# nizepart/Research-and-Development-of-Kubernetes-Operator-for-Machine-Learning-Pipelines

Measured on AMD Instinct MI355X. Metric: served_tokens_per_sec, higher is better.
Workload: dtype bf16

## Files before the change

### research-and-development-of-kubernetes-operator-for-machine-learning-pipelines_amd/ops/csrc/bindings.cpp

```cpp
#include <climits>
#include <cstdlib>
#include <string>
#include <torch/library.h>
#include <ATen/ATen.h>
#include <c10/hip/HIPStream.h>
#include <c10/core/DeviceGuard.h>
#include <cmath>

#include "launch.h"
#include "gemm_plan.h"

namespace {

using at::Tensor;

hipStream_t cur_stream() { return c10::hip::getCurrentHIPStream().stream(); }

void check_bf16(const Tensor& t, const char* name) {
  TORCH_CHECK(t.is_cuda(), name, " must be a GPU tensor");
  TORCH_CHECK(t.scalar_type() == at::kBFloat16, name, " must be bf16");
  TORCH_CHECK(t.is_contiguous(), name, " must be contiguous");
}
void check_i32(const Tensor& t, const char* name) {
  TORCH_CHECK(t.is_cuda(), name, " must be a GPU tensor");
// ... 403 lines not shown
std::vector<int64_t> gemm_route_env(int64_t M, int64_t N, int64_t K, int64_t op, int64_t cus, bool sk,
                                    int64_t n_groups, int64_t rows_per_group) {
  mlop::PlanEnv env = mlop::gemm_knobs();
  env.cus = (int)cus, env.sk = sk;
  return route_list(env, M, N, K, op, n_groups, rows_per_group);
}
std::vector<int64_t> gemm_tile_configs() {
  std::vector<int64_t> v;
  for (const mlop::TileCfg& t : mlop::kGemmTiles) v.insert(v.end(), {t.BM, t.BN, t.WM, t.WN, t.stages, t.setprio, t.rope});
  return v;
}

void check_a(const Tensor& a) {
  TORCH_CHECK(a.is_cuda() && a.scalar_type() == at::kBFloat16 && a.dim() == 2 && a.stride(1) == 1 &&
                  a.stride(0) % 8 == 0, "a must be bf16 [M, K], 16-B aligned rows");
}

mlop::RopeEpi rope_args(const Tensor& q_out, const Tensor& k_cache, const Tensor& v_cache, const Tensor& a,
                        const Tensor& w, const Tensor& pos, const Tensor& cos_sin, const Tensor& slots) {
  check_a(a);
  check_bf16(w, "w"); check_bf16(q_out, "q_out"); check_bf16(k_cache, "k_cache");
  check_bf16(v_cache, "v_cache"); check_i32(pos, "pos"); check_i32(slots, "slots");
  TORCH_CHECK(cos_sin.is_cuda() && cos_sin.scalar_type() == at::kFloat && cos_sin.is_contiguous(),
              "cos_sin f32");
  const int64_t M = a.size(0), K = a.size(1), N = w.size(0);
  TORCH_CHECK(w.dim() == 2 && w.size(1) == K && K % 64 == 0, "w [N, K], K % 64");
  TORCH_CHECK(q_out.dim() == 3 && k_cache.dim() == 4 && v_cache.dim() == 4, "ranks");
  const int64_t Hq = q_out.size(1), D = q_out.size(2), Hkv = k_cache.size(1), BS = k_cache.size(2);
  TORCH_CHECK(D == 128 && k_cache.size(3) == D && v_cache.sizes() == k_cache.sizes(),
              "head_dim 128; k and v [NB,Hkv,BS,D]");
  TORCH_CHECK(N == (Hq + 2 * Hkv) * D && q_out.size(0) == M, "qkv width / q_out rows");
  TORCH_CHECK(pos.numel() == M && slots.numel() == M, "pos/slots length");
  TORCH_CHECK(cos_sin.dim() == 2 && cos_sin.size(1) == D, "cos_sin [max_pos, D]");
  return mlop::RopeEpi{(uint16_t*)q_out.data_ptr(), (uint16_t*)k_cache.data_ptr(),
                       (uint16_t*)v_cache.data_ptr(), pos.data_ptr<int>(), cos_sin.data_ptr<float>(),
                       slots.data_ptr<int>(), (int)Hq, (int)Hkv, (int)BS};
}

void gemm(Tensor out, Tensor a, Tensor w, Tensor ws, int64_t epi) {
  TORCH_CHECK(a.is_cuda() && a.scalar_type() == at::kBFloat16 && a.dim() == 2 && a.stride(1) == 1,
              "a must be bf16 [M, K] with unit inner stride");
  check_bf16(w, "w");
  TORCH_CHECK(out.is_cuda() && out.scalar_type() == at::kBFloat16 && out.dim() == 2 &&
                  out.stride(1) == 1, "out must be bf16 [M, N]");
  const int64_t M = a.size(0), K = a.size(1), N = w.size(0);
  TORCH_CHECK(w.dim() == 2 && w.size(1) == K, "w must be [N, K]");
  TORCH_CHECK(K % 64 == 0, "K must be a multiple of 64");
  TORCH_CHECK(N % 8 == 0 && a.stride(0) % 8 == 0 && out.stride(0) % 8 == 0, "16-B aligned rows");
  TORCH_CHECK(epi == 0 || epi == 1, "epi");
  TORCH_CHECK(epi == 0 || N % 32 == 0, "silu_mul epilogue needs N % 32 == 0");
  TORCH_CHECK(out.size(0) == M && out.size(1) == (epi == 0 ? N : N / 2), "out shape");
  TORCH_CHECK(reinterpret_cast<uintptr_t>(a.data_ptr()) % 16 == 0 &&
                  reinterpret_cast<uintptr_t>(out.data_ptr()) % 16 == 0, "16-B aligned data");
  float* wsp = nullptr;
  int64_t wsn = 0;
  if (ws.defined() && ws.numel() > 0) {
    TORCH_CHECK(ws.is_cuda() && ws.scalar_type() == at::kFloat, "ws f32");
    wsp = ws.data_ptr<float>();
    wsn = ws.numel();
  }
  c10::DeviceGuard g(a.device());
  mlop::launch_gemm(a.data_ptr(), (int)a.stride(0), w.data_ptr(), (int)K, out.data_ptr(),
                    (int)out.stride(0), wsp, wsn, (int)M, (int)N, (int)K, (int)epi, cur_stream());
}

bool gemm_rope_cache(Tensor q_out, Tensor k_cache, Tensor v_cache, Tensor a, Tensor w, Tensor pos,
                     Tensor cos_sin, Tensor slots) {
  const mlop::RopeEpi re = rope_args(q_out, k_cache, v_cache, a, w, pos, cos_sin, slots);
  c10::DeviceGuard g(a.device());
// ... 16 lines not shown
  TORCH_CHECK(N % 128 == 0, "N % 128");
  check_ss(ss_out, M, N, "ss");
  c10::DeviceGuard g(a.device());
  return mlop::launch_gemm_chain(mlop::OP_CHAIN_RES_SS, a.data_ptr(), (int)a.stride(0), w.data_ptr(),
                                 residual.data_ptr(), (int)residual.stride(0), (int)M, (int)N, (int)K,
                                 mlop::RopeEpi{}, ss_out.data_ptr<float>(), 0.f, cur_stream());
}

bool gemm_rs(Tensor out, Tensor a, Tensor w, Tensor ss_in, double eps, int64_t epi) {
  check_a(a);
  check_bf16(w, "w"); check_bf16(out, "out");
  const int64_t M = a.size(0), K = a.size(1), N = w.size(0);
  TORCH_CHECK(w.dim() == 2 && w.size(1) == K, "w [N, K]");
  TORCH_CHECK(epi == 0 || epi == 1, "epi");
  TORCH_CHECK(out.dim() == 2 && out.size(0) == M && out.size(1) == (epi == 0 ? N : N / 2) && out.stride(1) == 1 &&
                  out.stride(0) % 8 == 0, "out [M, N or N/2]");
  TORCH_CHECK(K % 128 == 0, "K % 128");
  check_ss(ss_in, M, K, "ss");
  c10::DeviceGuard g(a.device());
  return mlop::launch_gemm_chain(mlop::OP_CHAIN_RS | (int)epi, a.data_ptr(), (int)a.stride(0), w.data_ptr(),
                                 out.data_ptr(), (int)out.stride(0), (int)M, (int)N, (int)K, mlop::RopeEpi{},
                                 ss_in.data_ptr<float>(), (float)eps, cur_stream());
}

bool gemm_rs_rope(Tensor q_out, Tensor k_cache, Tensor v_cache, Tensor a, Tensor w, Tensor pos, Tensor cos_sin,
                  Tensor slots, Tensor ss_in, double eps) {
  const mlop::RopeEpi re = rope_args(q_out, k_cache, v_cache, a, w, pos, cos_sin, slots);
  const int64_t M = a.size(0), K = a.size(1), N = w.size(0);
  TORCH_CHECK(K % 128 == 0, "K % 128");
  check_ss(ss_in, M, K, "ss");
  c10::DeviceGuard g(a.device());
  return mlop::launch_gemm_chain(mlop::OP_CHAIN_RS_ROPE, a.data_ptr(), (int)a.stride(0), w.data_ptr(), nullptr, 0,
                                 (int)M, (int)N, (int)K, re, ss_in.data_ptr<float>(), (float)eps, cur_stream());
}

bool gemm_add_rmsnorm(Tensor out, Tensor residual, Tensor a, Tensor w, Tensor norm_w, Tensor ws,
                      double eps) {
  check_a(a);
  check_bf16(w, "w"); check_bf16(out, "out"); check_bf16(residual, "residual");
  check_bf16(norm_w, "norm_w");
  const int64_t M = a.size(0), K = a.size(1), N = w.size(0);
  TORCH_CHECK(w.size(1) == K && K % 64 == 0 && N % 8 == 0, "w [N, K], K % 64");
  TORCH_CHECK(out.numel() == M * N && residual.numel() == M * N && norm_w.numel() == N, "shapes");
  TORCH_CHECK(ws.is_cuda() && ws.scalar_type() == at::kFloat, "ws f32");
  c10::DeviceGuard g(a.device());
  return mlop::launch_gemm_add_rmsnorm(a.data_ptr(), (int)a.stride(0), w.data_ptr(), out.data_ptr(),
                                       residual.data_ptr(), norm_w.data_ptr(), (float)eps,
                                       ws.data_ptr<float>(), ws.numel(), (int)M, (int)N, (int)K,
                                       cur_stream());
}

bool gemm_ws(Tensor out, Tensor a, Tensor w, int64_t epi, bool rs, double eps) {
  check_a(a);
  check_bf16(w, "w"); check_bf16(out, "out");
  const int64_t M = a.size(0), K = a.size(1), N = w.size(0);
  TORCH_CHECK(w.dim() == 2 && w.size(1) == K && w.stride(0) == K, "w [N, K] contiguous");
  TORCH_CHECK(epi == 0 || epi == 1 || epi == 5, "epi 0 / 1 / 5");
  TORCH_CHECK(out.dim() == 2 && out.size(0) == M && out.size(1) == (epi == 1 ? N / 2 : N) && out.stride(1) == 1,
              "out [M, N or N/2]");
  TORCH_CHECK(!(rs && epi == 5), "residual form has no row scale");
  if (!mlop::ws_takes(mlop::gemm_live_env(), (int)M, (int)N, (int)K, (int)epi)) return false;
  c10::DeviceGuard g(a.device());
  mlop::launch_ws(a.data_ptr(), (int)a.stride(0), w.data_ptr(), (int)K, out.data_ptr(), (int)out.stride(0), (int)M,
                  (int)N, (int)K, (int)epi, rs, mlop::RopeEpi{}, (float)eps, cur_stream());
  return true;
}
// ... 561 lines not shown
  m.def("decode_chain_max_m() -> int", &decode_chain_max_m);
  m.def("gemm_ws_plan(int rb, int u, int nt) -> ()", &gemm_ws_plan);
  m.def("gemm_ws_small_m(int set=-1) -> int", &knob<mlop::gemm_ws_small_m>);
  m.def("gemm_ws_rope_m(int set=-1) -> int", &knob<mlop::gemm_ws_rope_m>);
  m.def("flash_persist(int set=-1) -> int", &knob<mlop::flash_persist>);
  m.def("flash_stream(int set=-1) -> int", &knob<mlop::flash_stream>);
  m.def("gemm_grouped_balance(int set=-1) -> int", &knob<mlop::gemm_grouped_balance>);
  m.def("gemm_grouped_order(int set=-1) -> int", &knob<mlop::gemm_grouped_order>);
  m.def("moe_mid_tok(int set=-1) -> int", &knob<mlop::moe_mid_tok>);
  m.def("gemm_mid_chain(int set=-1) -> int", &knob<mlop::gemm_mid_chain>);
  m.def("mid_chain_ok(int M, int N, int K, int epi) -> bool", &mid_chain_ok);
  m.def("moe_mid_max_tokens(int set=-1) -> int", &knob<mlop::moe_mid_max_tokens>);
  m.def("gemm_grouped_plan(int bm, int bn, int stages, int splits) -> ()", &gemm_grouped_plan);
  m.def("gemm_dense_plan(int variant, int bm, int bn, int splits, int stages=0) -> ()", &gemm_dense_plan);
  m.def("gemm_small_stages(int set=-1) -> int", &knob<mlop::gemm_small_stages>);
  m.def("gemm_small_tile(int set=-1) -> int", &knob<mlop::gemm_small_tile>);
  m.def("gemm_sk_mode(int set=-1) -> int", &knob<mlop::gemm_sk_mode>);
  m.def("gemm_sk_reserve() -> bool", &gemm_sk_reserve);
  m.def("gemm_sk_workgroups(int M, int N, int K) -> int", &gemm_sk_workgroups);
  m.def("vmm_supported(int device) -> bool", &vmm_supported);
  m.def("vmm_granularity(int device) -> int", &vmm_granularity);
  m.def("vmm_arena(int bytes, int device) -> Tensor", &vmm_arena);
  m.def("vmm_map_chunks(Tensor flat, int region_stride, int n_regions, int chunk_bytes, int first, "
        "int count, bool async_) -> bool", &vmm_map_chunks);
  m.def("vmm_chunks_ready(Tensor flat) -> int", &vmm_chunks_ready);
  m.def("vmm_error(Tensor flat) -> int", &vmm_error);
  m.def("gemm_rope_supported(int M, int N, int K) -> bool", &gemm_rope_supported);
  m.def("w4_chain_ok(int M, int N, int K) -> bool", &w4_chain_ok);
  m.def("chain_ok(int M, int N, int K, int epi) -> bool", &chain_ok);
  m.def("gemm_route(int M, int N, int K, int op, int n_groups=0, int rows_per_group=0) -> int[]", &gemm_route);
  m.def("gemm_route_env(int M, int N, int K, int op, int cus, bool sk, int n_groups=0, int rows_per_group=0) -> int[]", &gemm_route_env);
  m.def("gemm_tile_configs() -> int[]", &gemm_tile_configs);
  m.def("gemm_res_ss(Tensor(a!) residual, Tensor a, Tensor w, Tensor(b!) ss_out) -> bool");
  m.def("gemm_rs(Tensor(a!) out, Tensor a, Tensor w, Tensor ss_in, float eps, int epi) -> bool");
  m.def("gemm_rs_rope(Tensor(a!) q_out, Tensor(b!) k_cache, Tensor(c!) v_cache, Tensor a, Tensor w, "
        "Tensor pos, Tensor cos_sin, Tensor slots, Tensor ss_in, float eps) -> bool");
  m.def("gemm_rope_cache(Tensor(a!) q_out, Tensor(b!) k_cache, Tensor(c!) v_cache, Tensor a, Tensor w, "
        "Tensor pos, Tensor cos_sin, Tensor slots) -> bool");
  m.def("gemm(Tensor(a!) out, Tensor a, Tensor w, Tensor(b!) ws, int epi) -> ()");
  m.def("grouped_gemm(Tensor(a!) out, Tensor a, Tensor w, Tensor offsets, int max_rows, "
        "int epi, Tensor? a_rows=None) -> ()");
  m.def("gemm_add_rmsnorm(Tensor(a!) out, Tensor(b!) residual, Tensor a, Tensor w, Tensor norm_w, "
        "Tensor(c!) ws, float eps) -> bool");
  m.def("gemv_chain_supported(int M, int N, int K, int epi) -> bool", &gemv_chain_supported);
  m.def("moe_route(Tensor(a!) topw, Tensor(b!) topi, Tensor logits) -> ()");
  m.def("moe_permute(Tensor(a!) xp, Tensor(b!) offsets, Tensor(c!) src, Tensor(d!) inv, Tensor x, "
        "Tensor topi, int e0, int n_local) -> ()");
  m.def("moe_combine(Tensor(a!) out, Tensor y, Tensor inv, Tensor topw) -> ()");
  m.def("moe_dispatch_small(Tensor(a!) topw, Tensor(b!) topi, Tensor(c!) xp, Tensor(d!) offsets, Tensor(e!) src, "
        "Tensor(f!) inv, Tensor(g!) x, Tensor router_w, int e0, int n_local, Tensor? pro_y=None, "
        "Tensor(h!)? pro_res=None, Tensor? pro_w=None, float pro_eps=0.0) -> bool");
  m.def("moe_dispatch_mid(Tensor(a!) topw, Tensor(b!) topi, Tensor(c!) offsets, Tensor(d!) arow, Tensor(e!) inv, "
        "Tensor(f!) x, Tensor router_w, int e0, int n_local, Tensor? pro_y=None, Tensor(g!)? pro_res=None, "
        "Tensor? pro_w=None, float pro_eps=0.0) -> bool");
  m.def("moe_down_combine_add_rmsnorm(Tensor(a!) out, Tensor(b!) residual, Tensor(c!) y, Tensor a, Tensor w2, "
        "Tensor offsets, int max_rows, Tensor inv, Tensor topw, Tensor norm_w, float eps) -> bool");
  m.def("moe_combine_add_rmsnorm(Tensor(a!) out, Tensor(b!) residual, Tensor y, Tensor inv, Tensor topw, "
        "Tensor norm_w, float eps) -> bool");
  m.def("argmax(Tensor(a!) out, Tensor logits) -> ()");
  m.def("sample(Tensor(a!) out, Tensor logits, Tensor temps, Tensor top_ks, Tensor top_ps, "
        "Tensor uniform, bool full) -> ()");
  m.def("penalty_reset(Tensor(a!) table, int slot, int vocab, Tensor prompt_ids, Tensor output_ids) -> ()");
  m.def("penalty_update(Tensor(a!) table, int vocab, Tensor slots, Tensor tokens) -> ()");
  m.def("grammar_mask(Tensor(a!) logits, Tensor arena, Tensor base, Tensor rows, Tensor state) -> ()");
  m.def("grammar_advance(Tensor arena, int vocab, Tensor base, Tensor rows, Tensor(a!) state, Tensor tokens) -> ()");
  m.def("apply_penalties(Tensor(a!) logits, Tensor table, Tensor slots, Tensor rep, Tensor freq, "
// ... 24 lines not shown
        "int nparts, int window=0) -> ()");
  m.def("rope_cache_fp8(Tensor(a!) q_out, Tensor(b!) k_cache, Tensor(c!) v_cache, Tensor(d!) k_scale, "
        "Tensor(e!) v_scale, Tensor qkv, Tensor pos, Tensor cos_sin, Tensor slots) -> ()");
  m.def("rope_cache_qkn(Tensor(a!) q_out, Tensor(b!) k_cache, Tensor(c!) v_cache, Tensor qkv, Tensor pos, "
        "Tensor cos_sin, Tensor slots, Tensor q_w, Tensor k_w, float eps) -> ()");
  m.def("rope_cache_qkn_fp8(Tensor(a!) q_out, Tensor(b!) k_cache, Tensor(c!) v_cache, Tensor(d!) k_scale, "
        "Tensor(e!) v_scale, Tensor qkv, Tensor pos, Tensor cos_sin, Tensor slots, Tensor q_w, Tensor k_w, "
        "float eps) -> ()");
  m.def("paged_attention_fp8(Tensor(a!) out, Tensor(b!) part_o, Tensor(c!) part_ml, Tensor(d!) part_sem, Tensor q, "
        "Tensor k_cache, Tensor v_cache, Tensor k_scale, Tensor v_scale, Tensor block_tables, Tensor tile_seq, "
        "Tensor tile_q0, Tensor q_start, Tensor q_len, Tensor ctx_len, float scale, int part_tokens, "
        "int nparts) -> ()");
}

TORCH_LIBRARY_IMPL(mlop, CUDA, m) {
  m.impl("rmsnorm", &rmsnorm);
  m.impl("add_rmsnorm", &add_rmsnorm);
  m.impl("rope_cache", &rope_cache);
  m.impl("silu_mul", &silu_mul);
  m.impl("embedding", &embedding);
  m.impl("lora_shrink", &lora_shrink);
  m.impl("lora_expand_add", &lora_expand_add);
  m.impl("paged_attention", &paged_attention);
  m.impl("rope_cache_fp8", &rope_cache_fp8);
  m.impl("rope_cache_qkn", &rope_cache_qkn);
  m.impl("rope_cache_qkn_fp8", &rope_cache_qkn_fp8);
  m.impl("paged_attention_fp8", &paged_attention_fp8);
  m.impl("flash_prefill", &flash_prefill);
  m.impl("gemm", &gemm);
  m.impl("gemm_ws", &gemm_ws);
  m.impl("grouped_gemm", &grouped_gemm);
  m.impl("gemm_add_rmsnorm", &gemm_add_rmsnorm);
  m.impl("gemm_res_ss", &gemm_res_ss);
  m.impl("gemm_rs", &gemm_rs);
  m.impl("gemm_rs_rope", &gemm_rs_rope);
  m.impl("gemm_rope_cache", &gemm_rope_cache);
  m.impl("moe_route", &moe_route);
  m.impl("moe_dispatch_small", &moe_dispatch_small);
  m.impl("moe_dispatch_mid", &moe_dispatch_mid);
  m.impl("moe_down_combine_add_rmsnorm", &moe_down_combine_add_rmsnorm);
  m.impl("moe_combine_add_rmsnorm", &moe_combine_add_rmsnorm);
  m.impl("moe_permute", &moe_permute);
  m.impl("moe_combine", &moe_combine);
  m.impl("argmax", &argmax);
  m.impl("sample", &sample);
  m.impl("penalty_reset", &penalty_reset);
  m.impl("penalty_update", &penalty_update);
  m.impl("grammar_mask", &grammar_mask);
  m.impl("grammar_advance", &grammar_advance);
  m.impl("apply_penalties", &apply_penalties);
  m.impl("token_logprobs", &token_logprobs);
  m.impl("spec_accept", &spec_accept);
  m.impl("spec_propose", &spec_propose);
  m.impl("pool_accumulate", &pool_accumulate);
  m.impl("pool_finish", &pool_finish);
  m.impl("car_all_reduce", &car_all_reduce);
  m.impl("car_all_reduce_add", &car_all_reduce_add);
  m.impl("car_broadcast", &car_broadcast);
  m.impl("car_all_gather", &car_all_gather);
  m.impl("ep_dispatch", &ep_dispatch);
  m.impl("ep_combine", &ep_combine);
}
```

### research-and-development-of-kubernetes-operator-for-machine-learning-pipelines_amd/ops/csrc/gemm_w4.hip

```cpp
#include "common.h"
#include "launch.h"
#include "gemm_plan.h"
#include "gemm_w4_asm.h"

#include <type_traits>
#include <utility>

namespace mlop {

namespace {
enum { W4_NONE = 0, W4_SILU_MUL = 1, W4_ROPE = 3, W4_ADD_SS = 4, W4_RS = 8 };
using i32x4 = __attribute__((ext_vector_type(4))) int;
typedef __attribute__((address_space(3))) uint16_t lds_u16;

__device__ __forceinline__ i32x4 make_srd(const void* p) {
  const uint64_t a = (uint64_t)p;
  i32x4 r;
  r.x = __builtin_amdgcn_readfirstlane((int)(uint32_t)a);
  r.y = __builtin_amdgcn_readfirstlane((int)(uint32_t)(a >> 32));
  r.z = 0x7fffffff;
  r.w = 0x00020000;
  return r;
}

// ... 142 lines not shown
#define MLOP_W4H_OPERANDS                                                                                        \
  : [fa0_0] "=&v"(fa0_0), [fa0_1] "=&v"(fa0_1), [fa0_2] "=&v"(fa0_2), [fa0_3] "=&v"(fa0_3),                      \
    [fb0_0] "=&v"(fb0_0), [fb0_1] "=&v"(fb0_1), [fb0_2] "=&v"(fb0_2), [fb0_3] "=&v"(fb0_3),                      \
    [fb0_4] "=&v"(fb0_4), [fb0_5] "=&v"(fb0_5), [fb0_6] "=&v"(fb0_6), [fb0_7] "=&v"(fb0_7),                      \
    [fa1_0] "=&v"(fa1_0), [fa1_1] "=&v"(fa1_1), [fa1_2] "=&v"(fa1_2), [fa1_3] "=&v"(fa1_3),                      \
    [fb1_0] "=&v"(fb1_0), [fb1_1] "=&v"(fb1_1), [fb1_2] "=&v"(fb1_2), [fb1_3] "=&v"(fb1_3),                      \
    [fb1_4] "=&v"(fb1_4), [fb1_5] "=&v"(fb1_5), [fb1_6] "=&v"(fb1_6), [fb1_7] "=&v"(fb1_7),                      \
    [rA0] "+v"(rA0), [rA1] "+v"(rA1), [rB0] "+v"(rB0), [rB1] "+v"(rB1), [koff] "+s"(koff), [dbase] "+s"(dbase), \
    [iter] "+s"(iter), [m0save] "=&s"(m0save)                                                                    \
  : [vo0] "v"(vo[0]), [vo1] "v"(vo[1]), [vo2] "v"(vo[2]), [vo3] "v"(vo[3]), [vo4] "v"(vo[4]), [vo5] "v"(vo[5]), \
    [vo6] "v"(vo[6]), [vo7] "v"(vo[7]), [vo8] "v"(vo[8]), [vo9] "v"(vo[9]), [vo10] "v"(vo[10]),                 \
    [vo11] "v"(vo[11]), [vn0] "v"(vn[0]), [vn1] "v"(vn[1]), [vn2] "v"(vn[2]), [vn3] "v"(vn[3]),                 \
    [vn4] "v"(vn[4]), [vn5] "v"(vn[5]), [vn6] "v"(vn[6]), [vn7] "v"(vn[7]), [vn8] "v"(vn[8]), [vn9] "v"(vn[9]), \
    [vn10] "v"(vn[10]), [vn11] "v"(vn[11]), [srdA] "s"(srdA), [srdB] "s"(srdB), [k128] "s"(k128),               \
    [first] "s"(s_first), [has_next] "s"(s_next)                                                                 \
  : "memory", "scc", MLOP_W4_AGPR_CLOBBERS
    constexpr int NQ = NS + (RS ? 2 : 0);
    if constexpr (BMT == 256) {
      static_assert(NQ == 32 || NQ == 16 || NQ == 34 || NQ == 18, "one generated K-loop per VMEM count");
      if constexpr (NQ == 32) asm volatile(MLOP_W4_KLOOP_S32_P0_ASM MLOP_W4_OPERANDS);
      else if constexpr (NQ == 16) asm volatile(MLOP_W4_KLOOP_S16_P0_ASM MLOP_W4_OPERANDS);
      else if constexpr (NQ == 34) asm volatile(MLOP_W4_KLOOP_S34_P0_ASM MLOP_W4_OPERANDS);
      else asm volatile(MLOP_W4_KLOOP_S18_P0_ASM MLOP_W4_OPERANDS);
    } else {
      static_assert(NQ == 16 || NQ == 8 || NQ == 18 || NQ == 10, "one generated K-loop per VMEM count");
      if constexpr (NQ == 16) asm volatile(MLOP_W4H_KLOOP_S16_ASM MLOP_W4H_OPERANDS);
      else if constexpr (NQ == 8) asm volatile(MLOP_W4H_KLOOP_S8_ASM MLOP_W4H_OPERANDS);
      else if constexpr (NQ == 18) asm volatile(MLOP_W4H_KLOOP_S18_ASM MLOP_W4H_OPERANDS);
      else asm volatile(MLOP_W4H_KLOOP_S10_ASM MLOP_W4H_OPERANDS);
    }
#undef MLOP_W4_OPERANDS
#undef MLOP_W4H_OPERANDS

    const int lr = wm * (BMT / 2) + (lane & 15), qd = lane >> 4;
    const bool part = it >= n_dp;
    const int sidx = part ? it - n_dp : 0;
    const auto rs_other = __builtin_amdgcn_make_buffer_rsrc(part ? ws + (size_t)(sidx ^ 1) * 65536 : (float*)C, 0,
                                                           65536 * 4, 0x00020000);
    if (part) {
      const int tt = sidx >> 1;
      const auto rs_own = __builtin_amdgcn_make_buffer_rsrc(ws + (size_t)sidx * 65536, 0, 65536 * 4, 0x00020000);
      auto put = [&](auto I_) {
        constexpr int I = decltype(I_)::value;
        float v[32];
        read_block<I>(v);
#pragma unroll
        for (int q4 = 0; q4 < 8; ++q4)
          __builtin_amdgcn_raw_buffer_store_b128(
              u32x4{__float_as_uint(v[4 * q4]), __float_as_uint(v[4 * q4 + 1]), __float_as_uint(v[4 * q4 + 2]),
                    __float_as_uint(v[4 * q4 + 3])},
              rs_own, (uint32_t)(((I * 8 + q4) * 256 + tid) * 16), 0, 16 );
      };
      unroll<NI>(put);
      asm volatile("s_waitcnt vmcnt(0)" ::: "memory");
      __syncthreads();
      int* flag = reinterpret_cast<int*>(smem);
      if (tid == 0) {
        const int tk = __hip_atomic_fetch_add(cnt + tt, 1, __ATOMIC_RELAXED, __HIP_MEMORY_SCOPE_AGENT);
        if (tk == 1) __hip_atomic_store(cnt + tt, 0, __ATOMIC_RELAXED, __HIP_MEMORY_SCOPE_AGENT);
        flag[0] = tk == 1;
      }
      __syncthreads();
      const int last = flag[0];
      __syncthreads();
      if (!last) break;
    }
    auto fetch = [&](auto I_, float (&v)[32]) {
// ... 5 lines not shown
          u32x4 o[4];
#pragma unroll
          for (int q4 = 0; q4 < 4; ++q4)
            o[q4] = __builtin_bit_cast(u32x4, __builtin_amdgcn_raw_buffer_load_b128(
                                                  rs_other, (uint32_t)(((I * 8 + b4 + q4) * 256 + tid) * 16), 0, 16 ));
#pragma unroll
          for (int q4 = 0; q4 < 4; ++q4)
#pragma unroll
            for (int e = 0; e < 4; ++e) v[4 * (b4 + q4) + e] += __uint_as_float(o[q4][e]);
        }
      }
      if constexpr (RS) {
        const float f = rsqrtf(rinv_lds[wid * 128 + 16 * I + (lane & 15)] * re.ss_inv_k + re.ss_eps);
#pragma unroll
        for (int e = 0; e < 32; ++e) v[e] *= f;
      }
    };
    const int odd = qd & 1, half = qd >> 1;
    auto swap_f = [&](const float* x, const float* y, float (&lo)[4], float (&hi)[4]) {
#pragma unroll
      for (int r = 0; r < 4; ++r) {
        const auto sw2 = __builtin_amdgcn_permlane16_swap(__float_as_uint(x[r]), __float_as_uint(y[r]), false, false);
        lo[r] = __uint_as_float(sw2[0]);
        hi[r] = __uint_as_float(sw2[1]);
      }
    };
    auto swap_pair = [&](const float* x, const float* y, u32x4& out) {
      float lo[4], hi[4];
      swap_f(x, y, lo, hi);
      out = u32x4{pack2(lo[0], lo[1]), pack2(lo[2], lo[3]), pack2(hi[0], hi[1]), pack2(hi[2], hi[3])};
    };
    if constexpr (BASE == W4_ROPE) {
      constexpr int D = 128, HALF = 64;
      const bool r_nt = (re.ws_nt & 8) != 0;
      auto put16 = [&](uint16_t* p, const u32x4& v) {
        if (r_nt) __builtin_nontemporal_store(v, reinterpret_cast<u32x4*>(p));
        else *reinterpret_cast<u32x4*>(p) = v;
      };
      const int head = (n0 + wn * 128) / D;
      const int n_rope = re.Hq + re.Hkv, n_all = re.Hq + 2 * re.Hkv;
      if (head >= n_all) {
      } else if (head >= n_rope) {
        const int kh = head - n_rope;
        int sl[NI];
#pragma unroll
        for (int I = 0; I < NI; ++I) {
          const int m = m0 + lr + I * 16;
          sl[I] = m < M ? re.slots[m] : -1;
        }
        auto vstore = [&](auto I_) {
          constexpr int I = decltype(I_)::value;
          float v[32];
          fetch(I_, v);
          u32x4 d[4];
#pragma unroll
          for (int pr = 0; pr < 4; ++pr) swap_pair(v + 8 * pr, v + 8 * pr + 4, d[pr]);
          const int slot = sl[I];
          if (slot < 0) return;
          uint16_t* dst = re.v_cache + (((size_t)(slot / re.BS) * re.Hkv + kh) * re.BS + slot % re.BS) * D;
#pragma unroll
          for (int pr = 0; pr < 4; ++pr)
            put16(dst + (2 * pr + odd) * 16 + 8 * half, d[pr]);
        };
        unroll<NI>(vstore);
      } else {
        const bool is_k = head >= re.Hq;
        int pp[NI], sl[NI];
#pragma unroll
        for (int I = 0; I < NI; ++I) {
          const int m = m0 + lr + I * 16;
          const bool ok = m < M;
          pp[I] = ok ? re.pos[m] : 0;
          sl[I] = ok && is_k ? re.slots[m] : -1;
        }
        const int c0 = 4 * qd;
        auto load_cs = [&](int I, float4 (&cs)[8]) {
          const float4* cr = reinterpret_cast<const float4*>(re.cos_sin + (size_t)pp[I] * D);
#pragma unroll
          for (int j = 0; j < 4; ++j) {
            cs[j] = cr[(j * 16 + c0) / 4];
            cs[4 + j] = cr[(HALF + j * 16 + c0) / 4];
          }
        };
        auto rstore = [&](auto I_, const float4 (&cs)[8], float4 (&nxt)[8]) {
          constexpr int I = decltype(I_)::value;
          if constexpr (I < NI - 1) load_cs(I + 1, nxt);
          float v[32];
          fetch(I_, v);
          float xo[4][4], yo[4][4];
#pragma unroll
          for (int j = 0; j < 4; ++j) {
            const float cv[4] = {cs[j].x, cs[j].y, cs[j].z, cs[j].w};
            const float sv[4] = {cs[4 + j].x, cs[4 + j].y, cs[4 + j].z, cs[4 + j].w};
#pragma unroll
            for (int r = 0; r < 4; ++r) {
              const float x = bf2f(f2bf(v[4 * j + r])), y = bf2f(f2bf(v[4 * (j + 4) + r]));
              xo[j][r] = x * cv[r] - y * sv[r];
              yo[j][r] = y * cv[r] + x * sv[r];
            }
          }
          u32x4 d[4];
          swap_pair(xo[0], xo[1], d[0]);
          swap_pair(xo[2], xo[3], d[1]);
          swap_pair(yo[0], yo[1], d[2]);
          swap_pair(yo[2], yo[3], d[3]);
          const int m = m0 + lr + I * 16;
          if (m >= M) return;
          uint16_t* dst;
          if (!is_k) {
            dst = re.q_out + ((size_t)m * re.Hq + head) * D;
          } else {
            const int slot = sl[I];
            if (slot < 0) return;
            dst = re.k_cache + (((size_t)(slot / re.BS) * re.Hkv + (head - re.Hq)) * re.BS + slot % re.BS) * D;
          }
#pragma unroll
          for (int b = 0; b < 4; ++b)
            put16(dst + (b >> 1) * HALF + ((b & 1) * 2 + odd) * 16 + 8 * half, d[b]);
        };
        float4 csa[8], csb[8];
        load_cs(0, csa);
        unroll<NI>([&](auto I_) {
          if constexpr (decltype(I_)::value % 2 == 0) rstore(I_, csa, csb);
          else rstore(I_, csb, csa);
        });
      }
    } else {
      const int col_w = BASE == W4_NONE ? n0 + wn * 128 : (n0 + wn * 128) / 2;
      const bool c_nt = (re.ws_nt & 2) != 0;
      const int n_groups = N >> 7, g_out = (n0 + wn * 128) >> 7;
      const auto rs_sso = __builtin_amdgcn_make_buffer_rsrc((void*)re.ss_out, 0, ADD ? (int)((uint32_t)M * n_groups * 4u) : 0,
                                                            0x00020000);
      auto store = [&](auto I_) {
        constexpr int I = decltype(I_)::value;
        float v[32];
        fetch(I_, v);
        const uint32_t row_off = (uint32_t)(m0 + lr + I * 16) * (uint32_t)ldc * 2u;
        if constexpr (BASE == W4_SILU_MUL) {
          float o[16];
#pragma unroll
          for (int jp = 0; jp < 4; ++jp)
#pragma unroll
            for (int r = 0; r < 4; ++r) o[4 * jp + r] = silu_bf(v[8 * jp + r]) * bf2f(f2bf(v[8 * jp + 4 + r]));
#pragma unroll
          for (int pr = 0; pr < 2; ++pr) {
            u32x4 d;
            swap_pair(o + 8 * pr, o + 8 * pr + 4, d);
            const int col = col_w + (2 * pr + odd) * 16 + 8 * half;
            if (c_nt) __builtin_amdgcn_raw_buffer_store_b128(d, srdC, row_off + col * 2, 0, 2 );
            else __builtin_amdgcn_raw_buffer_store_b128(d, srdC, row_off + col * 2, 0, 0);
          }
        } else {
#pragma unroll
          for (int pr = 0; pr < 4; ++pr) {
            u32x4 d;
            swap_pair(v + 8 * pr, v + 8 * pr + 4, d);
            const int col = col_w + (2 * pr + odd) * 16 + 8 * half;
            if (c_nt) __builtin_amdgcn_raw_buffer_store_b128(d, srdC, row_off + col * 2, 0, 2 );
            else __builtin_amdgcn_raw_buffer_store_b128(d, srdC, row_off + col * 2, 0, 0);
// ... 92 lines not shown
  auto kern = gemm_w4_kernel<EPI, BMT>;
  static bool attr = false;
  if (!attr) {
    (void)hipFuncSetAttribute((const void*)kern, hipFuncAttributeMaxDynamicSharedMemorySize, (int)lds);
    attr = true;
  }
  const int gx = (N + 255) / 256, gy = (M + BMT - 1) / BMT;
  constexpr int group_m = 1024 / BMT;
  const int gm = std::max(1, std::min(group_m, gy));
  const int T = gx * gy;
  int n_dp = T, n_items = T;
  float* ws = nullptr;
  int* cnt = nullptr;
  int cus = 256;
  if (gemm_w4_split_ok(gemm_live_env(), T, K / 64)) {
    int c2 = 0;
    if (gemm_sk_scratch(&ws, &cnt, &c2)) {
      n_dp = T - T % c2;
      n_items = n_dp + 2 * (T % c2);
    }
  }
  int grid = n_items;
  if (!gemm_sk_available(&cus) || cus <= 0) {
    static int cu_count[16] = {};
    int dev = 0;
    (void)hipGetDevice(&dev);
    if (dev >= 0 && dev < 16 && cu_count[dev] == 0)
      (void)hipDeviceGetAttribute(&cu_count[dev], hipDeviceAttributeMultiprocessorCount, dev);
    cus = (dev >= 0 && dev < 16 && cu_count[dev] > 0) ? cu_count[dev] : 256;
  }
  grid = std::min(grid, cus);
  RopeEpi re2 = re;
  re2.ws_nt = gemm_slab_nt(-1);
  if constexpr ((EPI & W4_ADD_SS) != 0) {
    float* w2 = nullptr;
    int c3 = 0;
    if (!gemm_sk_scratch(&w2, &re2.ss_cnt, &c3)) return false;
  }
  kern<<<grid, 256, lds, st>>>(A, lda, B, ldb, C, ldc, M, N, K, gx, gy, gm, re2, n_dp, n_items, ws, cnt);
  return true;
}

template <int BMT>
static bool run_w4_h(int epi, const uint16_t* A, int lda, const uint16_t* B, int ldb, uint16_t* C, int ldc, int M,
                     int N, int K, hipStream_t st, const RopeEpi& re) {
  switch (epi) {
    case W4_NONE: return run_w4_t<W4_NONE, BMT>(A, lda, B, ldb, C, ldc, M, N, K, st, re);
    case W4_SILU_MUL: return run_w4_t<W4_SILU_MUL, BMT>(A, lda, B, ldb, C, ldc, M, N, K, st, re);
    case W4_ROPE: return run_w4_t<W4_ROPE, BMT>(A, lda, B, ldb, C, ldc, M, N, K, st, re);
    case W4_ADD_SS: return run_w4_t<W4_ADD_SS, BMT>(A, lda, B, ldb, C, ldc, M, N, K, st, re);
    case W4_NONE | W4_RS: return run_w4_t<W4_NONE | W4_RS, BMT>(A, lda, B, ldb, C, ldc, M, N, K, st, re);
    case W4_SILU_MUL | W4_RS: return run_w4_t<W4_SILU_MUL | W4_RS, BMT>(A, lda, B, ldb, C, ldc, M, N, K, st, re);
    case W4_ROPE | W4_RS: return run_w4_t<W4_ROPE | W4_RS, BMT>(A, lda, B, ldb, C, ldc, M, N, K, st, re);
    default: return false;
  }
}

bool run_w4(int epi, const uint16_t* A, int lda, const uint16_t* B, int ldb, uint16_t* C, int ldc, int M, int N,
            int K, hipStream_t st, const RopeEpi& re, int bm) {
  if (bm == 128) return run_w4_h<128>(epi, A, lda, B, ldb, C, ldc, M, N, K, st, re);
  if (bm == 256) return run_w4_h<256>(epi, A, lda, B, ldb, C, ldc, M, N, K, st, re);
  return false;
}

}
```

### research-and-development-of-kubernetes-operator-for-machine-learning-pipelines_amd/ops/csrc/launch.h

```cpp
#pragma once

#include <string>
#include <hip/hip_runtime.h>
#include <stdint.h>
#include <algorithm>
#include <memory>

namespace mlop {

void launch_rmsnorm(void* out, const void* x, const void* w, float eps, int M, int H,
                    hipStream_t st);
void launch_add_rmsnorm(void* out, void* residual, const void* x, const void* w, float eps, int M,
                        int H, hipStream_t st);
void launch_rope_cache(void* q_out, void* k_cache, void* v_cache, const void* qkv, const int* pos,
                       const float* cos_sin, const int* slots, int T, int Hq, int Hkv, int D,
                       int qkv_stride, int BS, hipStream_t st);
void launch_silu_mul(void* out, const void* x, int M, int I, int interleaved, hipStream_t st);
void launch_device_delay(long long ticks, hipStream_t st);
void launch_lora_shrink(const void* x, int ldx, const void* A, float* tmp, const int* tok_slot,
                        const int* slot_rank, int T, int K, int GR, int R, int S, hipStream_t st);
void launch_lora_expand_add(void* y, int ldy, const float* tmp, const void* B, const uint8_t* tile_group,
                            const int* tok_slot, const int* slot_rank, int T, int N, int GR, int R, int S,
                            hipStream_t st);
void launch_embedding(void* out, const void* table, const long* ids, int T, int H, long vocab_start,
// ... 16 lines not shown
                               const uint16_t* k_w, float eps, hipStream_t st);
void launch_paged_attention_fp8(void* out, float* part_o, float* part_ml, const void* q, const void* kc,
                                const void* vc, const void* ks, const void* vs, const int* bt,
                                int bt_stride, const int* tile_seq, const int* tile_q0, const int* q_start,
                                const int* q_len, const int* ctx_len, int num_tiles, int Hq, int Hkv,
                                float scale_log2, int part_tokens, int nparts, int num_blocks, int* sem,
                                hipStream_t st);
int flash_persist(int set);
int flash_stream(int set);
int gemm_grouped_balance(int set);
int gemm_grouped_order(int set);
int moe_mid_tok(int set);
void launch_flash_prefill(void* out, const void* q, const void* kc, const void* vc, const int* bt,
                          int bt_stride, const int* ptile_seq, const int* ptile_q0,
                          const int* q_start, const int* q_len, const int* ctx_len, int num_ptiles,
                          int Hq, int Hkv, float scale_log2, int num_blocks, int window, hipStream_t st);
struct RopeEpi {
  uint16_t* q_out;
  uint16_t* k_cache;
  uint16_t* v_cache;
  const int* pos;
  const float* cos_sin;
  const int* slots;
  int Hq, Hkv, BS;
  const float* ss_in = nullptr;
  float* ss_out = nullptr;
  float* ss_tot = nullptr;
  int* ss_cnt = nullptr;
  float ss_inv_k = 0.f, ss_eps = 0.f;
  const int* a_rows = nullptr;
  int b_nt = 0;
  int ws_nt = 0;
  int mid_acq = 0;
};
void launch_rope_cache_slabs(const RopeEpi& re, const float* ws, int splits, int T, int N, hipStream_t st);
bool gemm_sk_scratch(float** ws, int** cnt, int* cus);
bool gemm_sk_available(int* cus);
bool run_w4(int epi, const uint16_t* A, int lda, const uint16_t* B, int ldb, uint16_t* C, int ldc, int M, int N,
            int K, hipStream_t st, const RopeEpi& re, int bm = 256);
bool launch_gemm_chain(int op, const void* A, int lda, const void* B, void* C, int ldc, int M, int N, int K,
                       const RopeEpi& rope, float* ss, float eps, hipStream_t st);
int gemm_small_nt(int set);
int attn_kv_nt(int set);
int gemm_slab_nt(int set);
bool gemm_sk_reserve();
void launch_gemv(const void* A, int lda, const void* B, int ldb, void* C, int ldc, int M, int N, int K,
                 int epi, hipStream_t st);
void launch_gemv_rope(const void* A, int lda, const void* B, int M, int N, int K, const RopeEpi& re,
                      hipStream_t st);
struct NormPro {
  float eps = 0.f;
};
void gemm_ws_plan(int rb, int u, int nt);
void launch_ws(const void* A, int lda, const void* B, int ldb, void* C, int ldc, int M, int N, int K, int epi,
               bool rs, const RopeEpi& re, float eps, hipStream_t st);
void launch_gemv_rs(const void* A, int lda, const void* B, void* C, int ldc, int M, int N, int K, int epi,
                    const RopeEpi& re, float eps, hipStream_t st);
void launch_gemv_res(const void* A, int lda, const void* B, void* residual, int M, int N, int K, hipStream_t st);
void launch_gemv_grouped(const void* A, const void* B, void* C, const int* offsets, int n_groups, int M, int N,
                         int K, int epi, hipStream_t st);
bool launch_gemm_rope(const void* A, int lda, const void* B, int M, int N, int K, const RopeEpi& re,
                      hipStream_t st);
void launch_gemm(const void* A, int lda, const void* B, int ldb, void* C, int ldc, float* ws,
                 long ws_floats, int M, int N, int K, int epi, hipStream_t st);
bool launch_gemm_add_rmsnorm(const void* A, int lda, const void* B, void* out, void* residual,
                             const void* w, float eps, float* ws, long ws_floats, int M, int N,
// ... 109 lines not shown
```

Before: 38380.

## Use buffer loads/stores with OOB masking in W4 RoPE epilogue

```diff
diff --git a/research-and-development-of-kubernetes-operator-for-machine-learning-pipelines_amd/ops/csrc/bindings.cpp b/research-and-development-of-kubernetes-operator-for-machine-learning-pipelines_amd/ops/csrc/bindings.cpp
--- a/research-and-development-of-kubernetes-operator-for-machine-learning-pipelines_amd/ops/csrc/bindings.cpp
+++ b/research-and-development-of-kubernetes-operator-for-machine-learning-pipelines_amd/ops/csrc/bindings.cpp
@@ -459,9 +459,12 @@
   TORCH_CHECK(N == (Hq + 2 * Hkv) * D && q_out.size(0) == M, "qkv width / q_out rows");
   TORCH_CHECK(pos.numel() == M && slots.numel() == M, "pos/slots length");
   TORCH_CHECK(cos_sin.dim() == 2 && cos_sin.size(1) == D, "cos_sin [max_pos, D]");
-  return mlop::RopeEpi{(uint16_t*)q_out.data_ptr(), (uint16_t*)k_cache.data_ptr(),
-                       (uint16_t*)v_cache.data_ptr(), pos.data_ptr<int>(), cos_sin.data_ptr<float>(),
-                       slots.data_ptr<int>(), (int)Hq, (int)Hkv, (int)BS};
+  mlop::RopeEpi re{(uint16_t*)q_out.data_ptr(), (uint16_t*)k_cache.data_ptr(),
+                   (uint16_t*)v_cache.data_ptr(), pos.data_ptr<int>(), cos_sin.data_ptr<float>(),
+                   slots.data_ptr<int>(), (int)Hq, (int)Hkv, (int)BS};
+  re.kv_bytes = (long)k_cache.numel() * 2;
+  re.cs_bytes = (long)cos_sin.numel() * 4;
+  return re;
 }
 
 void gemm(Tensor out, Tensor a, Tensor w, Tensor ws, int64_t epi) {
@@ -544,6 +547,33 @@
   c10::DeviceGuard g(a.device());
   return mlop::launch_gemm_chain(mlop::OP_CHAIN_RS_ROPE, a.data_ptr(), (int)a.stride(0), w.data_ptr(), nullptr, 0,
                                  (int)M, (int)N, (int)K, re, ss_in.data_ptr<float>(), (float)eps, cur_stream());
+}
+
+bool w4_rope_cache(Tensor q_out, Tensor k_cache, Tensor v_cache, Tensor a, Tensor w, Tensor pos, Tensor cos_sin,
+                   Tensor slots, int64_t bm) {
+  const mlop::RopeEpi re = rope_args(q_out, k_cache, v_cache, a, w, pos, cos_sin, slots);
+  const int M = (int)a.size(0), K = (int)a.size(1), N = (int)w.size(0), lda = (int)a.stride(0);
+  if (!mlop::gemm_w4_ok(M, N, K, lda, K, 0)) return false;
+  c10::DeviceGuard g(a.device());
+  return mlop::run_w4(3, (const uint16_t*)a.data_ptr(), lda, (const uint16_t*)w.data_ptr(), K, nullptr, 0, M, N, K,
+                      cur_stream(), re, (int)bm);
+}
+bool w4_res_ss(Tensor residual, Tensor a, Tensor w, Tensor ss_out, int64_t bm) {
+  check_a(a);
+  check_bf16(w, "w"); check_bf16(residual, "residual");
+  const int64_t M = a.size(0), K = a.size(1), N = w.size(0);
+  TORCH_CHECK(w.dim() == 2 && w.size(1) == K, "w [N, K]");
+  TORCH_CHECK(residual.dim() == 2 && residual.size(0) == M && residual.size(1) == N && residual.stride(1) == 1 &&
+                  residual.stride(0) % 8 == 0, "residual [M, N]");
+  check_ss(ss_out, M, N, "ss");
+  const int lda = (int)a.stride(0), ldc = (int)residual.stride(0);
+  if (!mlop::gemm_w4_ok((int)M, (int)N, (int)K, lda, (int)K, ldc) || (M + bm - 1) / bm > mlop::kSkMaxWg) return false;
+  mlop::RopeEpi re{};
+  re.ss_out = ss_out.data_ptr<float>();
+  re.ss_tot = re.ss_out + (size_t)M * (N / 128);
+  c10::DeviceGuard g(a.device());
+  return mlop::run_w4(4, (const uint16_t*)a.data_ptr(), lda, (const uint16_t*)w.data_ptr(), (int)K,
+                      (uint16_t*)residual.data_ptr(), ldc, (int)M, (int)N, (int)K, cur_stream(), re, (int)bm);
 }
 
 bool gemm_add_rmsnorm(Tensor out, Tensor residual, Tensor a, Tensor w, Tensor norm_w, Tensor ws,
@@ -1171,6 +1201,9 @@
   m.def("gemm_route_env(int M, int N, int K, int op, int cus, bool sk, int n_groups=0, int rows_per_group=0) -> int[]", &gemm_route_env);
   m.def("gemm_tile_configs() -> int[]", &gemm_tile_configs);
   m.def("gemm_res_ss(Tensor(a!) residual, Tensor a, Tensor w, Tensor(b!) ss_out) -> bool");
+  m.def("w4_res_ss(Tensor(a!) residual, Tensor a, Tensor w, Tensor(b!) ss_out, int bm) -> bool");
+  m.def("w4_rope_cache(Tensor(a!) q_out, Tensor(b!) k_cache, Tensor(c!) v_cache, Tensor a, Tensor w, "
+        "Tensor pos, Tensor cos_sin, Tensor slots, int bm) -> bool");
   m.def("gemm_rs(Tensor(a!) out, Tensor a, Tensor w, Tensor ss_in, float eps, int epi) -> bool");
   m.def("gemm_rs_rope(Tensor(a!) q_out, Tensor(b!) k_cache, Tensor(c!) v_cache, Tensor a, Tensor w, "
         "Tensor pos, Tensor cos_sin, Tensor slots, Tensor ss_in, float eps) -> bool");
@@ -1261,6 +1294,8 @@
   m.impl("grouped_gemm", &grouped_gemm);
   m.impl("gemm_add_rmsnorm", &gemm_add_rmsnorm);
   m.impl("gemm_res_ss", &gemm_res_ss);
+  m.impl("w4_res_ss", &w4_res_ss);
+  m.impl("w4_rope_cache", &w4_rope_cache);
   m.impl("gemm_rs", &gemm_rs);
   m.impl("gemm_rs_rope", &gemm_rs_rope);
   m.impl("gemm_rope_cache", &gemm_rope_cache);
diff --git a/research-and-development-of-kubernetes-operator-for-machine-learning-pipelines_amd/ops/csrc/gemm_w4.hip b/research-and-development-of-kubernetes-operator-for-machine-learning-pipelines_amd/ops/csrc/gemm_w4.hip
--- a/research-and-development-of-kubernetes-operator-for-machine-learning-pipelines_amd/ops/csrc/gemm_w4.hip
+++ b/research-and-development-of-kubernetes-operator-for-machine-learning-pipelines_amd/ops/csrc/gemm_w4.hip
@@ -198,7 +198,9 @@
 #undef MLOP_W4_OPERANDS
 #undef MLOP_W4H_OPERANDS
 
-    const int lr = wm * (BMT / 2) + (lane & 15), qd = lane >> 4;
+    int lane_e = lane;
+    if constexpr (BASE == W4_ROPE) asm volatile("" : "+v"(lane_e));
+    const int lr = wm * (BMT / 2) + (lane_e & 15), qd = lane_e >> 4;
     const bool part = it >= n_dp;
     const int sidx = part ? it - n_dp : 0;
     const auto rs_other = __builtin_amdgcn_make_buffer_rsrc(part ? ws + (size_t)(sidx ^ 1) * 65536 : (float*)C, 0,
@@ -270,21 +272,51 @@
     };
     if constexpr (BASE == W4_ROPE) {
       constexpr int D = 128, HALF = 64;
+      constexpr uint32_t kOob = 0xffffff00u;
       const bool r_nt = (re.ws_nt & 8) != 0;
-      auto put16 = [&](uint16_t* p, const u32x4& v) {
-        if (r_nt) __builtin_nontemporal_store(v, reinterpret_cast<u32x4*>(p));
-        else *reinterpret_cast<u32x4*>(p) = v;
-      };
+      const bool wide = re.kv_bytes == 0;
       const int head = (n0 + wn * 128) / D;
       const int n_rope = re.Hq + re.Hkv, n_all = re.Hq + 2 * re.Hkv;
+      const uint32_t kvb = (uint32_t)re.kv_bytes;
+      const auto srdCS = __builtin_amdgcn_make_buffer_rsrc((void*)re.cos_sin, 0, (int)(uint32_t)re.cs_bytes, 0x00020000);
+      const auto srdPos = __builtin_amdgcn_make_buffer_rsrc((void*)re.pos, 0, (int)((uint32_t)M * 4u), 0x00020000);
+      const auto srdSl = __builtin_amdgcn_make_buffer_rsrc((void*)re.slots, 0, (int)((uint32_t)M * 4u), 0x00020000);
+      const uint32_t lane_b = (uint32_t)(odd * 16 + 8 * half) * 2u;
+      auto page_row = [&](int slot, int kh) {
+        const uint32_t s = (uint32_t)slot, bs = (uint32_t)re.BS;
+        return ((s / bs) * (uint32_t)re.Hkv + (uint32_t)kh) * bs + s % bs;
+      };
+      auto put_row = [&](auto WIDE_, auto NT_, const auto& srd, uint16_t* base, bool ok, uint32_t row,
+                         const u32x4 (&d)[4]) {
+        if constexpr (decltype(WIDE_)::value) {
+          if (!ok) return;
+          uint16_t* dst = base + (size_t)row * D + lane_b / 2;
+#pragma unroll
+          for (int b = 0; b < 4; ++b) {
+            u32x4* p = reinterpret_cast<u32x4*>(dst + (b >> 1) * HALF + (b & 1) * 32);
+            if (r_nt) __builtin_nontemporal_store(d[b], p);
+            else *p = d[b];
+          }
+        } else {
+          const uint32_t off = (ok ? row * 256u : kOob) + lane_b;
+#pragma unroll
+          for (int b = 0; b < 4; ++b) {
+            const uint32_t cb = (uint32_t)((b >> 1) * HALF + (b & 1) * 32) * 2u;
+            __builtin_amdgcn_raw_buffer_store_b128(d[b], srd, off + cb, 0, decltype(NT_)::value);
+          }
+        }
+      };
+      auto rope_heads = [&](auto WIDE_, auto NT_) {
+      constexpr bool WIDE = decltype(WIDE_)::value;
       if (head >= n_all) {
       } else if (head >= n_rope) {
         const int kh = head - n_rope;
+        const auto srdV = __builtin_amdgcn_make_buffer_rsrc((void*)re.v_cache, 0, (int)kvb, 0x00020000);
         int sl[NI];
 #pragma unroll
         for (int I = 0; I < NI; ++I) {
           const int m = m0 + lr + I * 16;
-          sl[I] = m < M ? re.slots[m] : -1;
+          sl[I] = (int)__builtin_amdgcn_raw_buffer_load_b32(srdSl, (uint32_t)m * 4u, 0, 0);
         }
         auto vstore = [&](auto I_) {
           constexpr int I = decltype(I_)::value;
@@ -294,35 +326,41 @@
 #pragma unroll
           for (int pr = 0; pr < 4; ++pr) swap_pair(v + 8 * pr, v + 8 * pr + 4, d[pr]);
           const int slot = sl[I];
-          if (slot < 0) return;
-          uint16_t* dst = re.v_cache + (((size_t)(slot / re.BS) * re.Hkv + kh) * re.BS + slot % re.BS) * D;
-#pragma unroll
-          for (int pr = 0; pr < 4; ++pr)
-            put16(dst + (2 * pr + odd) * 16 + 8 * half, d[pr]);
+          put_row(WIDE_, NT_, srdV, re.v_cache, slot >= 0 && m0 + lr + I * 16 < M, page_row(slot, kh), d);
         };
         unroll<NI>(vstore);
       } else {
         const bool is_k = head >= re.Hq;
+        uint16_t* const dbase = is_k ? re.k_cache : re.q_out;
+        const auto srdD = __builtin_amdgcn_make_buffer_rsrc(
+            (void*)dbase, 0, (int)(wide ? 0u : is_k ? kvb : (uint32_t)M * (uint32_t)re.Hq * 256u), 0x00020000);
         int pp[NI], sl[NI];
 #pragma unroll
         for (int I = 0; I < NI; ++I) {
           const int m = m0 + lr + I * 16;
-          const bool ok = m < M;
-          pp[I] = ok ? re.pos[m] : 0;
-          sl[I] = ok && is_k ? re.slots[m] : -1;
+          pp[I] = (int)__builtin_amdgcn_raw_buffer_load_b32(srdPos, (uint32_t)m * 4u, 0, 0);
+          sl[I] = (int)__builtin_amdgcn_raw_buffer_load_b32(srdSl, (uint32_t)m * 4u, 0, 0);
         }
         const int c0 = 4 * qd;
         auto load_cs = [&](int I, float4 (&cs)[8]) {
-          const float4* cr = reinterpret_cast<const float4*>(re.cos_sin + (size_t)pp[I] * D);
-#pragma unroll
-          for (int j = 0; j < 4; ++j) {
-            cs[j] = cr[(j * 16 + c0) / 4];
-            cs[4 + j] = cr[(HALF + j * 16 + c0) / 4];
+          if constexpr (WIDE) {
+            const float4* cr = reinterpret_cast<const float4*>(re.cos_sin + (size_t)pp[I] * D);
+#pragma unroll
+            for (int j = 0; j < 4; ++j) {
+              cs[j] = cr[(j * 16 + c0) / 4];
+              cs[4 + j] = cr[(HALF + j * 16 + c0) / 4];
+            }
+          } else {
+            const uint32_t off = (uint32_t)pp[I] * (uint32_t)(D * 4) + (uint32_t)c0 * 4u;
+#pragma unroll
+            for (int j = 0; j < 4; ++j) {
+              cs[j] = __builtin_bit_cast(float4, __builtin_amdgcn_raw_buffer_load_b128(srdCS, off + j * 64u, 0, 0));
+              cs[4 + j] = __builtin_bit_cast(float4, __builtin_amdgcn_raw_buffer_load_b128(srdCS, off + HALF * 4u + j * 64u, 0, 0));
+            }
           }
         };
-        auto rstore = [&](auto I_, const float4 (&cs)[8], float4 (&nxt)[8]) {
+        auto rstore = [&](auto I_, float4 (&cs)[8]) {
           constexpr int I = decltype(I_)::value;
-          if constexpr (I < NI - 1) load_cs(I + 1, nxt);
           float v[32];
           fetch(I_, v);
           float xo[4][4], yo[4][4];
@@ -333,36 +371,37 @@
 #pragma unroll
             for (int r = 0; r < 4; ++r) {
               const float x = bf2f(f2bf(v[4 * j + r])), y = bf2f(f2bf(v[4 * (j + 4) + r]));
-              xo[j][r] = x * cv[r] - y * sv[r];
-              yo[j][r] = y * cv[r] + x * sv[r];
+              if (RS && j >= 1) {
+                xo[j][r] = __builtin_fmaf(-y, sv[r], x * cv[r]);
+                yo[j][r] = __builtin_fmaf(y, cv[r], x * sv[r]);
+              } else {
+                xo[j][r] = __builtin_fmaf(x, cv[r], -(y * sv[r]));
+                yo[j][r] = __builtin_fmaf(x, sv[r], y * cv[r]);
+              }
             }
           }
+          if constexpr (I + 2 < NI) load_cs(I + 2, cs);
           u32x4 d[4];
           swap_pair(xo[0], xo[1], d[0]);
           swap_pair(xo[2], xo[3], d[1]);
           swap_pair(yo[0], yo[1], d[2]);
           swap_pair(yo[2], yo[3], d[3]);
           const int m = m0 + lr + I * 16;
-          if (m >= M) return;
-          uint16_t* dst;
-          if (!is_k) {
-            dst = re.q_out + ((size_t)m * re.Hq + head) * D;
-          } else {
-            const int slot = sl[I];
-            if (slot < 0) return;
-            dst = re.k_cache + (((size_t)(slot / re.BS) * re.Hkv + (head - re.Hq)) * re.BS + slot % re.BS) * D;
-          }
-#pragma unroll
-          for (int b = 0; b < 4; ++b)
-            put16(dst + (b >> 1) * HALF + ((b & 1) * 2 + odd) * 16 + 8 * half, d[b]);
+          put_row(WIDE_, NT_, srdD, dbase, m < M && (!is_k || sl[I] >= 0),
+                  is_k ? page_row(sl[I], head - re.Hq) : (uint32_t)m * (uint32_t)re.Hq + (uint32_t)head, d);
         };
         float4 csa[8], csb[8];
         load_cs(0, csa);
+        load_cs(1, csb);
         unroll<NI>([&](auto I_) {
-          if constexpr (decltype(I_)::value % 2 == 0) rstore(I_, csa, csb);
-          else rstore(I_, csb, csa);
+          if constexpr (decltype(I_)::value % 2 == 0) rstore(I_, csa);
+          else rstore(I_, csb);
         });
       }
+      };
+      if (wide) rope_heads(std::true_type{}, std::integral_constant<int, 0>{});
+      else if (r_nt) rope_heads(std::false_type{}, std::integral_constant<int, 2>{});
+      else rope_heads(std::false_type{}, std::integral_constant<int, 0>{});
     } else {
       const int col_w = BASE == W4_NONE ? n0 + wn * 128 : (n0 + wn * 128) / 2;
       const bool c_nt = (re.ws_nt & 2) != 0;
@@ -521,6 +560,12 @@
   grid = std::min(grid, cus);
   RopeEpi re2 = re;
   re2.ws_nt = gemm_slab_nt(-1);
+  if constexpr ((EPI & 3) == W4_ROPE) {
+    constexpr long lim = 0xffffff00l;
+    const bool fits = re.kv_bytes > 0 && re.kv_bytes <= lim && re.cs_bytes > 0 && re.cs_bytes <= lim &&
+                      (long)M * re.Hq * 256l <= lim;
+    if (!fits || (re2.ws_nt & 16)) re2.kv_bytes = 0;
+  }
   if constexpr ((EPI & W4_ADD_SS) != 0) {
     float* w2 = nullptr;
     int c3 = 0;
diff --git a/research-and-development-of-kubernetes-operator-for-machine-learning-pipelines_amd/ops/csrc/launch.h b/research-and-development-of-kubernetes-operator-for-machine-learning-pipelines_amd/ops/csrc/launch.h
--- a/research-and-development-of-kubernetes-operator-for-machine-learning-pipelines_amd/ops/csrc/launch.h
+++ b/research-and-development-of-kubernetes-operator-for-machine-learning-pipelines_amd/ops/csrc/launch.h
@@ -72,6 +72,7 @@
   int b_nt = 0;
   int ws_nt = 0;
   int mid_acq = 0;
+  long kv_bytes = 0, cs_bytes = 0;
 };
 void launch_rope_cache_slabs(const RopeEpi& re, const float* ws, int splits, int T, int N, hipStream_t st);
 bool gemm_sk_scratch(float** ws, int** cnt, int* cus);
```

Result: no change. 38380 (median of 2 runs) (-0.0%).
